# jwcalder/GraphLearningLayer

Hardware: NVIDIA B200
Metric: gll_fwd_bwd_calls_per_sec (higher is better)
Workload: dtype f32

## Files before the change

### graphlearninglayer_b200/csrc/knn.cu

```cuda
#include <math.h>
#include <stdlib.h>
#include <string.h>

#include <algorithm>
#include <vector>

#include <cuda_fp16.h>
#include <cuda_fp16.h>

#include "common.cuh"
#include "knn_common.cuh"

namespace gll {
namespace {

constexpr int BM = 128, BN = 128, BK = 16, PAD = 4;
constexpr int GEMM_THREADS = 256;
constexpr int LDS_A = BM + PAD, LDS_B = BN + PAD;

constexpr size_t gemm_smem_bytes() {
  return sizeof(float) * (2 * BK * LDS_A + 2 * BK * LDS_B) + sizeof(u64) * (BM * KC + BM * BN) +
         sizeof(float) * BM + sizeof(int) * BM;
}

// ... 190 lines not shown
  float* Bs = As + 2 * BK * LDS_A;
  u64* topk = reinterpret_cast<u64*>(Bs + 2 * BK * LDS_B);
  u64* pend = topk + BM * KC;
  float* thr = reinterpret_cast<float*>(pend + BM * BN);
  int* pcnt = reinterpret_cast<int*>(thr + BM);

  const int tid = threadIdx.x, lane = tid & 31, warp = tid >> 5;
  const int tx = tid & 15, ty = tid >> 4;
  const int row0 = row_begin + blockIdx.x * BM;
  const int split = blockIdx.y;
  int t_lo = 0, t_hi = n;
  if (SEG) {
    t_lo = __ldg(&win[row0].x);
    t_hi = __ldg(&win[min(row_end, row0 + BM) - 1].y);
  }
  const int c_begin = t_lo + split * cols_per_split;
  const int c_end = min(t_hi, c_begin + cols_per_split);

  for (int t = tid; t < BM * KC; t += GEMM_THREADS) topk[t] = KEY_INF;
  for (int t = tid; t < BM; t += GEMM_THREADS) {
    thr[t] = INFINITY;
    pcnt[t] = 0;
  }
  __syncthreads();

  const int ktiles = (d + BK - 1) / BK;
  for (int c0 = c_begin; c0 < c_end; c0 += BN) {
    float acc[8][8];
#pragma unroll
    for (int i = 0; i < 8; ++i)
#pragma unroll
      for (int j = 0; j < 8; ++j) acc[i][j] = 0.f;

    float4 ra[2], rb[2];
    load_tile_regs<VEC4>(X, n, d, row0, 0, tid, ra);
    load_tile_regs<VEC4>(X, n, d, c0, 0, tid, rb);
    store_tile_smem(As, LDS_A, tid, ra);
    store_tile_smem(Bs, LDS_B, tid, rb);
    __syncthreads();
    for (int kt = 0; kt < ktiles; ++kt) {
      const int cur = kt & 1;
      if (kt + 1 < ktiles) {
        load_tile_regs<VEC4>(X, n, d, row0, (kt + 1) * BK, tid, ra);
        load_tile_regs<VEC4>(X, n, d, c0, (kt + 1) * BK, tid, rb);
      }
      const float* A = As + cur * BK * LDS_A;
      const float* B = Bs + cur * BK * LDS_B;
#pragma unroll
      for (int kk = 0; kk < BK; ++kk) {
        float4 a0 = *reinterpret_cast<const float4*>(A + kk * LDS_A + ty * 4);
        float4 a1 = *reinterpret_cast<const float4*>(A + kk * LDS_A + 64 + ty * 4);
        float4 b0 = *reinterpret_cast<const float4*>(B + kk * LDS_B + tx * 4);
        float4 b1 = *reinterpret_cast<const float4*>(B + kk * LDS_B + 64 + tx * 4);
        float a[8] = {a0.x, a0.y, a0.z, a0.w, a1.x, a1.y, a1.z, a1.w};
        float b[8] = {b0.x, b0.y, b0.z, b0.w, b1.x, b1.y, b1.z, b1.w};
#pragma unroll
        for (int i = 0; i < 8; ++i)
#pragma unroll
          for (int j = 0; j < 8; ++j) acc[i][j] = fmaf(a[i], b[j], acc[i][j]);
      }
      if (kt + 1 < ktiles) {
        store_tile_smem(As + (cur ^ 1) * BK * LDS_A, LDS_A, tid, ra);
        store_tile_smem(Bs + (cur ^ 1) * BK * LDS_B, LDS_B, tid, rb);
      }
      __syncthreads();
    }

    float sqj[8];
    int gjv[8];
#pragma unroll
    for (int j = 0; j < 8; ++j) {
      int cc = (j < 4) ? tx * 4 + j : 64 + tx * 4 + (j - 4);
      gjv[j] = c0 + cc;
      sqj[j] = (gjv[j] < c_end) ? __ldg(sq + gjv[j]) : 0.f;
    }
#pragma unroll
    for (int i = 0; i < 8; ++i) {
      int rr = (i < 4) ? ty * 4 + i : 64 + ty * 4 + (i - 4);
      int gi = row0 + rr;
      if (gi >= row_end) continue;
      float t = thr[rr];
      float sqi = __ldg(sq + gi);
      int w_lo = 0, w_hi = n;
      if (SEG) {
        const int2 w = __ldg(win + gi);
        w_lo = w.x;
        w_hi = w.y;
      }
#pragma unroll
      for (int j = 0; j < 8; ++j) {
        if (gjv[j] < c_end && gjv[j] != gi && (!SEG || (gjv[j] >= w_lo && gjv[j] < w_hi))) {
          float dist = fmaf(-2.f, acc[i][j], sqi + sqj[j]);
          if (dist < t) {
            int p = atomicAdd(&pcnt[rr], 1);
            pend[rr * BN + p] = make_key(dist, gjv[j]);
          }
        }
      }
    }
    __syncthreads();
    for (int rr = warp * (BM / 8); rr < (warp + 1) * (BM / 8); ++rr) {
      int c = pcnt[rr];
      if (c > 0) {
        u64 mine = topk[rr * KC + lane];
        for (int t = 0; t < c; ++t) list_insert(mine, pend[rr * BN + t], lane);
        topk[rr * KC + lane] = mine;
        if (lane == KC - 1) thr[rr] = (mine == KEY_INF) ? INFINITY : key_dist(mine);
        if (lane == 0) pcnt[rr] = 0;
      }
    }
    __syncthreads();
  }

  for (int rr = warp * (BM / 8); rr < (warp + 1) * (BM / 8); ++rr) {
    int gi = row0 + rr;
    if (gi < row_end) cand[((size_t)gi * splits + split) * KC + lane] = topk[rr * KC + lane];
  }
}

}

namespace {

constexpr int RERANK_WARPS = 4;

template <bool VEC4>
__device__ __forceinline__ double exact_d2(const float* __restrict__ xi_s, const float* __restrict__ xj, int d,
                                           int lane) {
  double part = 0.0;
  if (VEC4) {
    const float4* a = reinterpret_cast<const float4*>(xi_s);
    const float4* b = reinterpret_cast<const float4*>(xj);
    int q = d >> 2;
#pragma unroll 4
    for (int t = lane; t < q; t += 32) {
      float4 u = a[t], v = __ldg(b + t);
      double d0 = (double)u.x - (double)v.x, d1 = (double)u.y - (double)v.y;
      double d2 = (double)u.z - (double)v.z, d3 = (double)u.w - (double)v.w;
      part += d0 * d0;
      part += d1 * d1;
      part += d2 * d2;
      part += d3 * d3;
    }
  } else {
#pragma unroll 4
    for (int t = lane; t < d; t += 32) {
      double df = (double)xi_s[t] - (double)__ldg(xj + t);
      part += df * df;
    }
  }
  return warp_sum(part);
}

__device__ __forceinline__ double exact_d2_reg(const double (&xr)[16], const float* __restrict__ xj, int q, int lane) {
  const float4* b = reinterpret_cast<const float4*>(xj);
  float4 v[4];
#pragma unroll
  for (int t = 0; t < 4; ++t) v[t] = (lane + 32 * t < q) ? __ldg(b + lane + 32 * t) : make_float4(0.f, 0.f, 0.f, 0.f);
  double part = 0.0;
#pragma unroll
  for (int t = 0; t < 4; ++t) {
    if (lane + 32 * t < q) {
      const double d0 = xr[4 * t + 0] - (double)v[t].x, d1 = xr[4 * t + 1] - (double)v[t].y;
      const double d2 = xr[4 * t + 2] - (double)v[t].z, d3 = xr[4 * t + 3] - (double)v[t].w;
      part += d0 * d0;
      part += d1 * d1;
      part += d2 * d2;
      part += d3 * d3;
    }
  }
  return warp_sum(part);
}

__device__ __forceinline__ double knn_err_bound(float err_coef, float sqi, const unsigned* __restrict__ small) {
  const double sqm = (double)__uint_as_float(small[0]), rho = (double)__uint_as_float(small[2]);
  const double xi = sqrt((double)sqi);
  const double rterm = (small[5] == 2u) ? rho * (xi + sqrt(sqm) + rho) : xi * rho;
  return (double)err_coef * ((double)sqi + sqm) + 2.0 * rterm * 1.000001;
}

template <bool VEC4>
__global__ void __launch_bounds__(RERANK_WARPS * 32)
knn_rerank_kernel(const float* __restrict__ X, const float* __restrict__ sq, const unsigned* __restrict__ sqmax_bits,
                  int n, int d, int k, int row_end, CandLayout lay, const u64* __restrict__ cand, float err_coef,
                  int* __restrict__ knn_idx, float* __restrict__ knn_dist, int* __restrict__ flag_count,
                  int* __restrict__ flag_rows, int force_rows) {
  extern __shared__ __align__(16) float xs[];
  const int lane = threadIdx.x & 31, warp = threadIdx.x >> 5;
  const int i = lay.row_begin + blockIdx.x * RERANK_WARPS + warp;
  if (i >= row_end) return;
  float* xi = xs + (size_t)warp * d;
  const bool use_reg = VEC4 && d <= 512;
  double xr[16];
  if (use_reg) {
    const float4* xrow = reinterpret_cast<const float4*>(X + (size_t)i * d);
#pragma unroll
    for (int t = 0; t < 4; ++t) {
      const float4 u = (lane + 32 * t < (d >> 2)) ? __ldg(xrow + lane + 32 * t) : make_float4(0.f, 0.f, 0.f, 0.f);
      xr[4 * t + 0] = (double)u.x;
      xr[4 * t + 1] = (double)u.y;
      xr[4 * t + 2] = (double)u.z;
      xr[4 * t + 3] = (double)u.w;
    }
  } else {
    for (int t = lane; t < d; t += 32) xi[t] = X[(size_t)i * d + t];
  }

  u64 mine = KEY_INF;
  int splits = lay.stride;
  if (lay.tc == 1 || lay.tc == 3) {
    int b0, b1;
    cand_owner_range(lay, (i - lay.row_begin) / lay.row_tile, b0, b1);
    splits = 2 * (b1 - b0 + 1);
  }
  if (splits == 1 && lay.tc == 0) {
    mine = cand[(size_t)i * lay.stride * KC + lane];
  } else {
    for (int s = 0; s < splits; ++s) {
      list_merge_set(mine, cand[((size_t)i * lay.stride + s) * KC + lane], lane);
    }
  }
  u64 last = __shfl_sync(FULL, mine, KC - 1);
  const float lower = (last == KEY_INF) ? INFINITY : key_dist(last);
  __syncwarp();

  const double errb = knn_err_bound(err_coef, sq[i], sqmax_bits);
  const u64 kth = __shfl_sync(FULL, mine, k - 2);
  const float cutoff = (kth == KEY_INF) ? INFINITY : (float)((double)key_dist(kth) + 2.0 * errb + 1e-30) * (1.f + 1e-6f);
  double myd2 = INFINITY;
  int myj = -1;
  for (int c = 0; c < KC; ++c) {
    u64 kc = __shfl_sync(FULL, mine, c);
    if (kc == KEY_INF) break;
    if (c > k - 2 && key_dist(kc) > cutoff) break;
    int j = key_idx(kc);
    double v = use_reg ? exact_d2_reg(xr, X + (size_t)j * d, d >> 2, lane) : exact_d2<VEC4>(xi, X + (size_t)j * d, d, lane);
    if (lane == c) {
      myd2 = v;
      myj = j;
    }
  }
  int rank = 0;
  for (int c = 0; c < KC; ++c) {
    double od = __shfl_sync(FULL, myd2, c);
    int oj = __shfl_sync(FULL, myj, c);
    if (oj >= 0 && (od < myd2 || (od == myd2 && oj < myj))) ++rank;
  }
  if (myj >= 0 && rank < k - 1) {
    knn_idx[(size_t)i * k + 1 + rank] = myj;
    knn_dist[(size_t)i * k + 1 + rank] = (float)sqrt(myd2);
  }
  if (lane == 0) {
    knn_idx[(size_t)i * k] = i;
    knn_dist[(size_t)i * k] = 0.f;
  }
  unsigned who = __ballot_sync(FULL, myj >= 0 && rank == k - 2);
  bool ok = false;
  if (who) {
    double dk = __shfl_sync(FULL, myd2, __ffs(who) - 1);
    ok = ((double)lower - errb > dk) || (lower == INFINITY);
  }
  if (i - lay.row_begin < force_rows) ok = false;
  if (!ok && lane == 0) {
    int p = atomicAdd(flag_count, 1);
    flag_rows[p] = i;
  }
}

constexpr int FB_WARPS = 8;

__device__ __forceinline__ void list_insert_d(double& md, int& mj, double xd, int xj, int lane) {
  bool lt = (md < xd) || (md == xd && mj < xj);
  int pos = __popc(__ballot_sync(FULL, lt));
  double pd = __shfl_up_sync(FULL, md, 1);
  int pj = __shfl_up_sync(FULL, mj, 1);
  if (lane > pos) {
    md = pd;
    mj = pj;
  } else if (lane == pos) {
    md = xd;
    mj = xj;
  }
}

__device__ __forceinline__ bool pair_less(double ad, int aj, double bd, int bj) { return ad < bd || (ad == bd && aj < bj); }
__device__ __forceinline__ void dlist_merge_sorted(double& md, int& mj, double od, int oj, int lane) {
  const double rd = __shfl_sync(FULL, od, 31 - lane);
  const int rj = __shfl_sync(FULL, oj, 31 - lane);
  if (pair_less(rd, rj, md, mj)) {
    md = rd;
    mj = rj;
  }
#pragma unroll
  for (int j = 16; j >= 1; j >>= 1) {
    const double pd = __shfl_xor_sync(FULL, md, j);
    const int pj = __shfl_xor_sync(FULL, mj, j);
    const bool keep_min = (lane & j) == 0;
    const bool p_less = pair_less(pd, pj, md, mj);
    if (p_less == keep_min) {
      md = pd;
      mj = pj;
    }
  }
}

template <bool VEC4>
__global__ void __launch_bounds__(FB_WARPS * 32)
knn_fallback_kernel(const float* __restrict__ X, int n, int d, int k, const int* __restrict__ flag_count,
                    const int* __restrict__ flag_rows, int* __restrict__ knn_idx, float* __restrict__ knn_dist,
                    int* __restrict__ info) {
  extern __shared__ __align__(16) float xs[];
  __shared__ double sd[FB_WARPS][32];
  __shared__ int sj[FB_WARPS][32];
  const int lane = threadIdx.x & 31, warp = threadIdx.x >> 5;
  const int nflag = *flag_count;
  if (blockIdx.x == 0 && threadIdx.x == 0 && info != nullptr) {
    info[GLL_INFO_KNN_FALLBACK_ROWS] = nflag;
    if (nflag > 0) atomicOr(&info[GLL_INFO_STATUS], GLL_STATUS_KNN_FALLBACK);
  }
  for (int f = blockIdx.x; f < nflag; f += gridDim.x) {
    const int i = flag_rows[f];
    for (int t = threadIdx.x; t < d; t += blockDim.x) xs[t] = X[(size_t)i * d + t];
    __syncthreads();
    double ex_d = -1.0;
    int ex_j = -1;
    for (int pass = 0; pass * 32 < k - 1; ++pass) {
      double md = INFINITY;
      int mj = 0x7fffffff;
      for (int j = warp; j < n; j += FB_WARPS) {
        if (j == i) continue;
        double v = exact_d2<VEC4>(xs, X + (size_t)j * d, d, lane);
        if (v > ex_d || (v == ex_d && j > ex_j)) list_insert_d(md, mj, v, j, lane);
      }
      sd[warp][lane] = md;
      sj[warp][lane] = mj;
      __syncthreads();
      if (warp == 0) {
        for (int w = 1; w < FB_WARPS; ++w)
          for (int t = 0; t < 32; ++t) {
            int xj = sj[w][t];
            if (xj == 0x7fffffff) break;
            list_insert_d(md, mj, sd[w][t], xj, lane);
          }
        const int slot = pass * 32 + lane;
        if (slot < k - 1 && mj != 0x7fffffff) {
          knn_idx[(size_t)i * k + 1 + slot] = mj;
          knn_dist[(size_t)i * k + 1 + slot] = (float)sqrt(md);
        }
        if (lane == 0 && pass == 0) {
          knn_idx[(size_t)i * k] = i;
          knn_dist[(size_t)i * k] = 0.f;
        }
        if (lane == 31) {
          sd[0][0] = md;
          sj[0][0] = mj;
        }
      }
      __syncthreads();
      ex_d = sd[0][0];
      ex_j = sj[0][0];
      __syncthreads();
    }
    __syncthreads();
  }
}

template <bool VEC4>
__global__ void __launch_bounds__(FB_WARPS * 32)
knn_fallback_scan_kernel(const float* __restrict__ X, int n, int d, int k, const int* __restrict__ flag_count,
                         const int* __restrict__ flag_rows, int* __restrict__ knn_idx, float* __restrict__ knn_dist,
                         int* __restrict__ info, double* __restrict__ part_d, int* __restrict__ part_j,
                         unsigned* __restrict__ ticket, const int2* __restrict__ win) {
  extern __shared__ __align__(16) float xs[];
  __shared__ double sd[FB_WARPS][32];
  __shared__ int sj[FB_WARPS][32];
  __shared__ int last_cta;
  const int lane = threadIdx.x & 31, warp = threadIdx.x >> 5;
  const int nflag = *flag_count;
  if (blockIdx.x == 0 && threadIdx.x == 0 && info != nullptr) {
    info[GLL_INFO_KNN_FALLBACK_ROWS] = nflag;
    if (nflag > 0) atomicOr(&info[GLL_INFO_STATUS], GLL_STATUS_KNN_FALLBACK);
  }
  if (nflag == 0) return;
  const int G = gridDim.x, C = max(1, min(128, G / nflag));
  const long long T = (long long)nflag * C;
  for (long long t = blockIdx.x; t < T; t += G) {
    const int f = (int)(t / C), c = (int)(t - (long long)f * C);
    const int i = flag_rows[f];
    const int2 w = (win != nullptr) ? win[i] : make_int2(0, n);
    const int j0 = w.x + (int)((long long)(w.y - w.x) * c / C), j1 = w.x + (int)((long long)(w.y - w.x) * (c + 1) / C);
    __syncthreads();
    for (int q = threadIdx.x; q < d; q += blockDim.x) xs[q] = X[(size_t)i * d + q];
    __syncthreads();
    double md = INFINITY, thr_d = INFINITY;
    int mj = 0x7fffffff, thr_j = 0x7fffffff;
    for (int jb = j0 + 4 * warp; jb < j1; jb += 4 * FB_WARPS) {
// ... 59 lines not shown
        }
#pragma unroll
        for (int u = 0; u < 4; ++u) dlist_merge_sorted(md, mj, ld[u], lj[u], lane);
      }
      if (lane < k - 1 && mj != 0x7fffffff) {
        knn_idx[(size_t)i * k + 1 + lane] = mj;
        knn_dist[(size_t)i * k + 1 + lane] = (float)sqrt(md);
      }
      if (lane == 0) {
        knn_idx[(size_t)i * k] = i;
        knn_dist[(size_t)i * k] = 0.f;
      }
    }
    return;
  }
  for (int f = 0; f < nflag; ++f) {
    const int i = flag_rows[f];
    double md = INFINITY;
    int mj = 0x7fffffff;
    for (int c0 = warp; c0 < C; c0 += 4 * FB_WARPS) {
      double ld[4];
      int lj[4];
#pragma unroll
      for (int u = 0; u < 4; ++u) {
        const int c = c0 + u * FB_WARPS;
        ld[u] = (c < C) ? __ldcg(part_d + ((size_t)f * C + c) * 32 + lane) : INFINITY;
        lj[u] = (c < C) ? __ldcg(part_j + ((size_t)f * C + c) * 32 + lane) : 0x7fffffff;
      }
#pragma unroll
      for (int u = 0; u < 4; ++u) dlist_merge_sorted(md, mj, ld[u], lj[u], lane);
    }
    __syncthreads();
    sd[warp][lane] = md;
    sj[warp][lane] = mj;
    __syncthreads();
    if (warp == 0) {
      for (int w = 1; w < FB_WARPS; ++w) dlist_merge_sorted(md, mj, sd[w][lane], sj[w][lane], lane);
      if (lane < k - 1 && mj != 0x7fffffff) {
        knn_idx[(size_t)i * k + 1 + lane] = mj;
        knn_dist[(size_t)i * k + 1 + lane] = (float)sqrt(md);
      }
      if (lane == 0) {
        knn_idx[(size_t)i * k] = i;
        knn_dist[(size_t)i * k] = 0.f;
      }
    }
  }
}


__global__ void __launch_bounds__(RERANK_WARPS * 32)
knn_merge_kernel(int row_end, CandLayout lay, const u64* __restrict__ cand, u64* __restrict__ merged, u64* __restrict__ excl) {
  const int lane = threadIdx.x & 31, warp = threadIdx.x >> 5;
  const int i = lay.row_begin + blockIdx.x * RERANK_WARPS + warp;
  if (i >= row_end) return;
  int splits = lay.stride;
  if (lay.tc == 1) {
    int b0, b1;
    cand_owner_range(lay, (i - lay.row_begin) / lay.row_tile, b0, b1);
    splits = 2 * (b1 - b0 + 1);
  }
  u64 mine = KEY_INF;
  for (int s = 0; s < splits; ++s) {
    list_merge_set(mine, cand[((size_t)i * lay.stride + s) * KC + lane], lane);
  }
  merged[(size_t)(i - lay.row_begin) * KC + lane] = mine;
  if (excl != nullptr && lane == KC - 1) excl[i] = mine;
}

template <bool VEC4>
__global__ void __launch_bounds__(RERANK_WARPS * 32)
knn_rerank64_kernel(const float* __restrict__ X, const float* __restrict__ sq, const unsigned* __restrict__ sqmax_bits, int n, int d,
                    int k, int row_begin, int row_end, const u64* __restrict__ m1, const u64* __restrict__ m2, float err_coef,
                    int* __restrict__ knn_idx, float* __restrict__ knn_dist, int* __restrict__ flag_count,
                    int* __restrict__ flag_rows) {
  extern __shared__ __align__(16) float xs[];
  const int lane = threadIdx.x & 31, warp = threadIdx.x >> 5;
  const int i = row_begin + blockIdx.x * RERANK_WARPS + warp;
  if (i >= row_end) return;
  float* xi = xs + (size_t)warp * d;
  for (int t = lane; t < d; t += 32) xi[t] = X[(size_t)i * d + t];
  __syncwarp();
  const u64 ca = m1[(size_t)(i - row_begin) * KC + lane];
  u64 cb = m2[(size_t)(i - row_begin) * KC + lane];
  const u64 last = __shfl_sync(FULL, cb, KC - 1);
  const float lower = (last == KEY_INF) ? INFINITY : key_dist(last);
  {
    bool dup = false;
    for (int c = 0; c < KC; ++c) {
      const u64 oa = __shfl_sync(FULL, ca, c);
      dup |= (oa != KEY_INF && cb != KEY_INF && key_idx(oa) == key_idx(cb));
    }
    if (dup) cb = KEY_INF;
  }
  double da = INFINITY, db = INFINITY;
  int ja = -1, jb = -1;
  for (int c = 0; c < 2 * KC; ++c) {
    const u64 kc = __shfl_sync(FULL, (c < KC) ? ca : cb, c & (KC - 1));
    if (kc == KEY_INF) continue;
    const int j = key_idx(kc);
    const double v = exact_d2<VEC4>(xi, X + (size_t)j * d, d, lane);
    if (lane == (c & (KC - 1))) {
      if (c < KC) {
        da = v;
        ja = j;
      } else {
        db = v;
        jb = j;
      }
    }
  }
  int ra = 0, rb = 0;
  for (int c = 0; c < 2 * KC; ++c) {
    const double od = __shfl_sync(FULL, (c < KC) ? da : db, c & (KC - 1));
    const int oj = __shfl_sync(FULL, (c < KC) ? ja : jb, c & (KC - 1));
    if (oj < 0) continue;
    ra += (od < da || (od == da && oj < ja)) ? 1 : 0;
    rb += (od < db || (od == db && oj < jb)) ? 1 : 0;
  }
  if (ja >= 0 && ra < k - 1) {
    knn_idx[(size_t)i * k + 1 + ra] = ja;
    knn_dist[(size_t)i * k + 1 + ra] = (float)sqrt(da);
  }
  if (jb >= 0 && rb < k - 1) {
    knn_idx[(size_t)i * k + 1 + rb] = jb;
    knn_dist[(size_t)i * k + 1 + rb] = (float)sqrt(db);
  }
  if (lane == 0) {
    knn_idx[(size_t)i * k] = i;
    knn_dist[(size_t)i * k] = 0.f;
  }
  const unsigned wa = __ballot_sync(FULL, ja >= 0 && ra == k - 2), wb = __ballot_sync(FULL, jb >= 0 && rb == k - 2);
  bool ok = false;
  if (wa | wb) {
    const double dk = wa ? __shfl_sync(FULL, da, __ffs(wa) - 1) : __shfl_sync(FULL, db, __ffs(wb) - 1);
    const double errb = knn_err_bound(err_coef, sq[i], sqmax_bits);
    ok = ((double)lower - errb > dk) || (lower == INFINITY);
  }
  if (!ok && lane == 0) {
    int p = atomicAdd(flag_count, 1);
    flag_rows[p] = i;
  }
}

}

int knn_fallback_grid() { return 2 * device_info().sms; }
size_t knn_fallback_scratch_bytes() { return align_up((size_t)knn_fallback_grid() * 32 * (sizeof(double) + sizeof(int)), 256); }

int knn_finish(const float* X, const float* sq, const unsigned* sqmax_bits, int n, int d, int k, int row_begin, int row_end,
               CandLayout lay, const u64* cand, float err_coef, int* knn_idx, float* knn_dist, int* flag_count, int* flag_rows,
               int* info, void* fb_scratch, cudaStream_t st, const int2* win) {
  const bool vec4 = (d % 4 == 0) && ((reinterpret_cast<uintptr_t>(X) & 15) == 0);
  size_t smem = sizeof(float) * (size_t)RERANK_WARPS * d;
  lay.row_begin = row_begin;
  int blocks = ceil_div(row_end - row_begin, RERANK_WARPS);
  int force_rows = 0;
  if (const char* e = getenv("GLL_B200_KNN_FORCE_FALLBACK")) force_rows = atoi(e);
  if (vec4) {
    if (smem > 48 * 1024)
      GLL_CUDA_CHECK(cudaFuncSetAttribute(knn_rerank_kernel<true>, cudaFuncAttributeMaxDynamicSharedMemorySize, (int)smem));
    {
      GLL_PROF(KID_RERANK, st);
      knn_rerank_kernel<true><<<blocks, RERANK_WARPS * 32, smem, st>>>(X, sq, sqmax_bits, n, d, k, row_end, lay, cand,
                                                                      err_coef, knn_idx, knn_dist, flag_count, flag_rows, force_rows);
    }
  } else {
    if (smem > 48 * 1024)
      GLL_CUDA_CHECK(cudaFuncSetAttribute(knn_rerank_kernel<false>, cudaFuncAttributeMaxDynamicSharedMemorySize, (int)smem));
    {
      GLL_PROF(KID_RERANK, st);
      knn_rerank_kernel<false><<<blocks, RERANK_WARPS * 32, smem, st>>>(X, sq, sqmax_bits, n, d, k, row_end, lay, cand,
                                                                       err_coef, knn_idx, knn_dist, flag_count, flag_rows, force_rows);
    }
  }
  GLL_LAUNCH_CHECK();
  size_t fsmem = sizeof(float) * (size_t)d;
  if (getenv("GLL_B200_KNN_DEBUG") != nullptr) return GLL_OK;
  {
    const int fblocks = knn_fallback_grid();
    double* part_d = reinterpret_cast<double*>(fb_scratch);
    int* part_j = reinterpret_cast<int*>(part_d + (size_t)fblocks * 32);
    unsigned* ticket = reinterpret_cast<unsigned*>(flag_count) + 7;
    GLL_PROF(KID_KNN_FALLBACK, st);
    if (vec4)
      knn_fallback_scan_kernel<true><<<fblocks, FB_WARPS * 32, fsmem, st>>>(X, n, d, k, flag_count, flag_rows, knn_idx, knn_dist, info,
                                                                           part_d, part_j, ticket, win);
    else
      knn_fallback_scan_kernel<false><<<fblocks, FB_WARPS * 32, fsmem, st>>>(X, n, d, k, flag_count, flag_rows, knn_idx, knn_dist, info,
                                                                            part_d, part_j, ticket, win);
  }
  GLL_LAUNCH_CHECK();
  return GLL_OK;
}

static int knn_finish64(const float* X, const float* sq, const unsigned* sqmax_bits, int n, int d, int k, int row_begin, int row_end,
                       const u64* m1, const u64* m2, float err_coef, int* knn_idx, float* knn_dist, int* flag_count,
                       int* flag_rows, int* info, cudaStream_t st) {
  const bool vec4 = (d % 4 == 0) && ((reinterpret_cast<uintptr_t>(X) & 15) == 0);
  const size_t smem = sizeof(float) * (size_t)RERANK_WARPS * d;
  const int blocks = ceil_div(row_end - row_begin, RERANK_WARPS);
  {
    GLL_PROF(KID_RERANK, st);
    if (vec4) {
      if (smem > 48 * 1024)
        GLL_CUDA_CHECK(cudaFuncSetAttribute(knn_rerank64_kernel<true>, cudaFuncAttributeMaxDynamicSharedMemorySize, (int)smem));
      knn_rerank64_kernel<true><<<blocks, RERANK_WARPS * 32, smem, st>>>(X, sq, sqmax_bits, n, d, k, row_begin, row_end, m1, m2,
                                                                          err_coef, knn_idx, knn_dist, flag_count, flag_rows);
    } else {
      if (smem > 48 * 1024)
        GLL_CUDA_CHECK(cudaFuncSetAttribute(knn_rerank64_kernel<false>, cudaFuncAttributeMaxDynamicSharedMemorySize, (int)smem));
      knn_rerank64_kernel<false><<<blocks, RERANK_WARPS * 32, smem, st>>>(X, sq, sqmax_bits, n, d, k, row_begin, row_end, m1, m2,
                                                                           err_coef, knn_idx, knn_dist, flag_count, flag_rows);
    }
  }
  GLL_LAUNCH_CHECK();
  const size_t fsmem = sizeof(float) * (size_t)d;
  const int fblocks = device_info().sms;
  if (getenv("GLL_B200_KNN_DEBUG") != nullptr) return GLL_OK;
  {
    GLL_PROF(KID_KNN_FALLBACK, st);
    if (vec4)
      knn_fallback_kernel<true><<<fblocks, FB_WARPS * 32, fsmem, st>>>(X, n, d, k, flag_count, flag_rows, knn_idx, knn_dist, info);
    else
      knn_fallback_kernel<false><<<fblocks, FB_WARPS * 32, fsmem, st>>>(X, n, d, k, flag_count, flag_rows, knn_idx, knn_dist, info);
  }
  GLL_LAUNCH_CHECK();
  return GLL_OK;
}

static int simt_splits(int n, int rows, int* cols_per_split) {
  int row_tiles = ceil_div(rows, BM), col_tiles = ceil_div(n, BN);
  int want = ceil_div(2 * device_info().sms, row_tiles);
  want = max(1, min(want, min(col_tiles, KNN_MAX_SPLITS)));
  int tiles_per = ceil_div(col_tiles, want);
  *cols_per_split = tiles_per * BN;
  return ceil_div(col_tiles, tiles_per);
}

static int cand_stride(int n, int d, int row_begin, int row_end) {
  const TcPlan plan = knn_tc_plan(n, d, row_begin, row_end);
  if (plan.ok) return plan.max_splits;
  int cps;
  return simt_splits(n, row_end - row_begin, &cps);
}

static size_t knn_common_bytes(int n, int d, size_t rows, int stride) {
  size_t b = 0;
  b += align_up(sizeof(float) * (size_t)n, 256);
  b += 256;
  b += align_up(sizeof(u64) * rows * (size_t)stride * KC, 256);
  b += align_up(sizeof(int) * rows, 256);
  b += knn_tc_ws_upper(n, d);
  b += align_up(sizeof(unsigned) * (size_t)n, 256);
  b += align_up(sizeof(float) * (size_t)n, 256);
  b += knn_fallback_scratch_bytes() + 256;
  return b;
}

size_t knn_ws_bytes(int n, int d, int k, int row_begin, int row_end) {
  const size_t rows = (size_t)(row_end - row_begin);
  size_t b = knn_common_bytes(n, d, rows, cand_stride(n, d, row_begin, row_end));
  if (k > KC + 1) b += 2 * align_up(sizeof(u64) * rows * KC, 256) + align_up(sizeof(u64) * (size_t)n, 256);
  return b + 1024;
}

namespace {

struct KnnBufs {
  float* sq;
  unsigned* small;
  int* flag_count;
  u64* cand;
  int* flag_rows;
  char* tc_ws;
  unsigned* thr_g;
  float* rscale;
  void* fb_scratch;
};

KnnBufs knn_carve(Carver& cv, int n, int d, int row_begin, int row_end, int stride) {
  const int rows = row_end - row_begin;
  KnnBufs b;
  b.sq = cv.take<float>(n);
  b.small = cv.take<unsigned>(64);
  b.flag_count = reinterpret_cast<int*>(b.small + 1);
  b.cand = cv.take<u64>((size_t)rows * stride * KC) - (size_t)row_begin * stride * KC;
  b.flag_rows = cv.take<int>(rows);
  b.tc_ws = cv.take<char>(knn_tc_ws_upper(n, d));
  b.thr_g = cv.take<unsigned>(n);
  b.rscale = cv.take<float>(n);
  b.fb_scratch = cv.take<char>(knn_fallback_scratch_bytes());
  const char* sh = getenv("GLL_B200_KNN_SHARE");
  if (sh && sh[0] == '0') b.thr_g = nullptr;
  return b;
}

CandLayout layout_of(const TcPlan& plan, int row_begin, const int* gfirst = nullptr) {
  CandLayout lay;
  lay.stride = plan.max_splits;
  lay.tc = plan.aligned ? 2 : (gfirst != nullptr ? 3 : 1);
  lay.row_tile = 128 * plan.rstep;
  lay.col_tiles = plan.col_tiles;
  lay.grid = plan.grid;
  lay.units = plan.units;
  lay.row_begin = row_begin;
  lay.gfirst = gfirst;
  return lay;
}

CandLayout simt_layout(int splits) {
  CandLayout lay;
  lay.stride = splits;
  lay.tc = 0;
  lay.row_tile = lay.col_tiles = lay.grid = 0;
  lay.units = 0;
  lay.row_begin = 0;
  lay.gfirst = nullptr;
  return lay;
}

float simt_err_coef(int d) {
  const double u = 5.9604644775390625e-8;
  return (float)(((double)d * u / (1.0 - (double)d * u) + 4.0 * u) * 1.0001);
}

int launch_simt(const float* X, const float* sq, int n, int d, int cps, int splits, u64* cand, int row_begin, int row_end,
                const int2* win, cudaStream_t st) {
  const bool vec4 = (d % 4 == 0) && ((reinterpret_cast<uintptr_t>(X) & 15) == 0);
  const bool seg = win != nullptr;
  auto kern = vec4 ? (seg ? knn_gemm_topk_kernel<true, true> : knn_gemm_topk_kernel<true, false>)
                   : (seg ? knn_gemm_topk_kernel<false, true> : knn_gemm_topk_kernel<false, false>);
  const dim3 grid(ceil_div(row_end - row_begin, BM), splits);
  const size_t smem = gemm_smem_bytes();
  GLL_CUDA_CHECK(set_max_dynamic_smem_once((const void*)kern, (int)smem));
  {
    GLL_PROF(KID_GRAM_TOPK, st);
    kern<<<grid, GEMM_THREADS, smem, st>>>(X, sq, n, d, cps, splits, cand, row_begin, row_end, win);
  }
  GLL_LAUNCH_CHECK();
  return GLL_OK;
}

}

static int launch_split_f16(const float* X, int n, int d, const TcPlan& plan, float* sq, unsigned* small, char* tc_ws, float* rscale,
                            unsigned* thr_g, cudaStream_t st) {
  __half* H = reinterpret_cast<__half*>(tc_ws);
  __half* L = (plan.passes == 2) ? reinterpret_cast<__half*>(tc_ws + align_up((size_t)n * plan.d_pad * 2, 256)) : nullptr;
  const int grid = ceil_div((long long)ceil_div(n, plan.d_pad <= 1024 ? 2 : 1) * 32, 256);
  if (plan.d_pad <= 256)
    sqnorm_split_f16_kernel<4><<<grid, 256, 0, st>>>(X, n, d, plan.d_pad, sq, small, H, L, rscale, thr_g);
  else if (plan.d_pad <= 512)
    sqnorm_split_f16_kernel<8><<<grid, 256, 0, st>>>(X, n, d, plan.d_pad, sq, small, H, L, rscale, thr_g);
  else if (plan.d_pad <= 1024)
    sqnorm_split_f16_kernel<16><<<grid, 256, 0, st>>>(X, n, d, plan.d_pad, sq, small, H, L, rscale, thr_g);
  else
    sqnorm_split_f16_kernel<0><<<grid, 256, 0, st>>>(X, n, d, plan.d_pad, sq, small, H, L, rscale, thr_g);
  GLL_LAUNCH_CHECK();
  return GLL_OK;
}

static int launch_norms(const float* X, int n, int d, const TcPlan& plan, const KnnBufs& b, cudaStream_t st) {
  GLL_PROF(KID_SQNORM, st);
  if (plan.ok) return launch_split_f16(X, n, d, plan, b.sq, b.small, b.tc_ws, b.rscale, b.thr_g, st);
  sqnorm_kernel<<<ceil_div((long long)n * 32, 256), 256, 0, st>>>(X, n, d, b.sq, b.small);
  GLL_LAUNCH_CHECK();
  return GLL_OK;
}

int knn_debug_gram_tile(const float* X, int n, int d, int row_tile, int col_tile, float* acc_out, float* rscale_out, void* ws,
                        size_t ws_bytes, cudaStream_t st) {
  GLL_REQUIRE(X && acc_out && rscale_out && ws, "null pointer");
  GLL_REQUIRE(n >= 256 && d >= 1, "the tensor-core path needs n >= 256");
  if (ws_bytes < knn_ws_bytes(n, d, 25, 0, n)) {
    set_error("workspace too small: %zu < %zu", ws_bytes, knn_ws_bytes(n, d, 25, 0, n));
    return GLL_ERR_WORKSPACE;
  }
  const TcPlan plan = knn_tc_plan(n, d, 0, n);
  GLL_REQUIRE(plan.ok, "tensor-core plan not available for this shape");
  GLL_REQUIRE(row_tile >= 0 && row_tile * 128 < n && col_tile >= 0 && col_tile * 256 < n, "tile out of range");
  Carver cv(ws, ws_bytes);
  float* sq = cv.take<float>(n);
  unsigned* small = cv.take<unsigned>(64);
  char* tc_ws = cv.take<char>(knn_tc_ws_upper(n, d));
  float* rscale = cv.take<float>(n);
  GLL_CUDA_CHECK(cudaMemsetAsync(small, 0, 256, st));
  const int rcs = launch_split_f16(X, n, d, plan, sq, small, tc_ws, rscale, nullptr, st);
  if (rcs) return rcs;
  GLL_CUDA_CHECK(cudaMemcpyAsync(rscale_out, rscale, sizeof(float) * (size_t)n, cudaMemcpyDeviceToDevice, st));
  return knn_tc_debug_tile(plan, n, tc_ws, row_tile, col_tile, acc_out, st);
}

int knn_run(const float* X, int n, int d, int k, int row_begin, int row_end, int* knn_idx, float* knn_dist, int* info,
            void* ws, size_t ws_bytes, cudaStream_t st) {
  GLL_REQUIRE(X && knn_idx && knn_dist && ws, "null pointer");
  GLL_REQUIRE(n >= k && k >= 2 && k <= 2 * KC, "need n >= k and 2 <= k <= 64");
  GLL_REQUIRE(d >= 1, "d must be positive");
  GLL_REQUIRE(0 <= row_begin && row_begin < row_end && row_end <= n, "bad row range");
  if (ws_bytes < knn_ws_bytes(n, d, k, row_begin, row_end)) {
    set_error("kNN workspace too small: %zu < %zu", ws_bytes, knn_ws_bytes(n, d, k, row_begin, row_end));
    return GLL_ERR_WORKSPACE;
  }
  const int rows = row_end - row_begin;
  Carver cv(ws, ws_bytes);
  const KnnBufs kb = knn_carve(cv, n, d, row_begin, row_end, cand_stride(n, d, row_begin, row_end));
  float* sq = kb.sq;
  unsigned* small = kb.small;
  unsigned* sqmax_bits = small;
  int* flag_count = kb.flag_count;
  u64* cand = kb.cand;
  int* flag_rows = kb.flag_rows;
  char* tc_ws = kb.tc_ws;
  unsigned* thr_g = kb.thr_g;
  float* rscale = kb.rscale;

  CandLayout lay;
  float err_coef;
  const TcPlan plan = knn_tc_plan(n, d, row_begin, row_end);
  GLL_CUDA_CHECK(cudaMemsetAsync(small, 0, 256, st));
  {
    const int rcs = launch_norms(X, n, d, plan, kb, st);
    if (rcs) return rcs;
  }

  if (k > KC + 1) {
    GLL_REQUIRE(plan.ok, "k > 33 needs the tensor-core path (n >= 256, row range starting on a multiple of 128)");
    u64* merged1 = cv.take<u64>((size_t)rows * KC);
    u64* merged2 = cv.take<u64>((size_t)rows * KC);
    u64* excl = cv.take<u64>(n);
    lay = layout_of(plan, row_begin);
    const int mblocks = ceil_div(rows, RERANK_WARPS);
    int rc = knn_tc_candidates(X, sq, rscale, small, n, d, row_end, plan, tc_ws, cand, nullptr, thr_g, st);
    if (rc) return rc;
    {
      GLL_PROF(KID_RERANK, st);
      knn_merge_kernel<<<mblocks, RERANK_WARPS * 32, 0, st>>>(row_end, lay, cand, merged1, excl);
    }
    GLL_LAUNCH_CHECK();
    rc = knn_tc_candidates(X, sq, rscale, small, n, d, row_end, plan, tc_ws, cand, excl, nullptr, st);
    if (rc) return rc;
    {
      GLL_PROF(KID_RERANK, st);
      knn_merge_kernel<<<mblocks, RERANK_WARPS * 32, 0, st>>>(row_end, lay, cand, merged2, nullptr);
    }
    GLL_LAUNCH_CHECK();
    return knn_finish64(X, sq, sqmax_bits, n, d, k, row_begin, row_end, merged1, merged2, knn_tc_err_coef(d, plan.passes), knn_idx, knn_dist,
                        flag_count, flag_rows, info, st);
  }
  if (plan.ok) {
    int rc = knn_tc_candidates(X, sq, rscale, small, n, d, row_end, plan, tc_ws, cand, nullptr, thr_g, st);
    if (rc) return rc;
    lay = layout_of(plan, row_begin);
    err_coef = knn_tc_err_coef(d, plan.passes);
  } else {
    int cps;
    const int splits = simt_splits(n, rows, &cps);
    const int rc = launch_simt(X, sq, n, d, cps, splits, cand, row_begin, row_end, nullptr, st);
    if (rc) return rc;
    lay = simt_layout(splits);
    err_coef = simt_err_coef(d);
  }
  return knn_finish(X, sq, sqmax_bits, n, d, k, row_begin, row_end, lay, cand, err_coef, knn_idx, knn_dist, flag_count, flag_rows,
                    info, kb.fb_scratch, st);
}


namespace {

// ... 288 lines not shown
```

### graphlearninglayer_b200/csrc/knn_common.cuh

```cuda
#pragma once
#include <vector>

#include "common.cuh"

namespace gll {

typedef unsigned long long u64;
constexpr int KC = 32;
constexpr int KNN_MAX_SPLITS = 32;
constexpr u64 KEY_INF = ~0ull;

__device__ __forceinline__ u64 make_key(float dist, int j) {
  return ((u64)float_to_ordered(dist) << 32) | (uint32_t)j;
}
__device__ __forceinline__ float key_dist(u64 k) { return ordered_to_float((uint32_t)(k >> 32)); }
__device__ __forceinline__ int key_idx(u64 k) { return (int)(uint32_t)k; }

__device__ __forceinline__ void list_insert(u64& mine, u64 x, int lane) {
  int pos = __popc(__ballot_sync(FULL, mine < x));
  u64 prev = __shfl_up_sync(FULL, mine, 1);
  if (lane > pos)
    mine = prev;
  else if (lane == pos)
    mine = x;
}

__device__ __forceinline__ void key_cmpx(u64& k, int j, bool keep_min) {
  const u64 o = __shfl_xor_sync(FULL, k, j);
  const bool less = k < o;
  k = (less == keep_min) ? k : o;
}
__device__ __forceinline__ void key_sort32(u64& k, int lane) {
#pragma unroll
  for (int w = 2; w <= 32; w <<= 1) {
#pragma unroll
    for (int j = w >> 1; j >= 1; j >>= 1) {
      const bool up = (lane & w) == 0;
      key_cmpx(k, j, ((lane & j) == 0) == up);
    }
  }
}
__device__ __forceinline__ void list_merge_set(u64& mine, u64 c, int lane) {
  unsigned m = __ballot_sync(FULL, c < __shfl_sync(FULL, mine, KC - 1));
  if (m == 0) return;
  if (__popc(m) > 6) {
    key_sort32(c, lane);
    const u64 r = __shfl_sync(FULL, c, 31 - lane);
    mine = (r < mine) ? r : mine;
#pragma unroll
    for (int j = 16; j >= 1; j >>= 1) key_cmpx(mine, j, (lane & j) == 0);
    return;
  }
  while (m) {
    const int t = __ffs(m) - 1;
    m &= m - 1;
    const u64 x = __shfl_sync(FULL, c, t);
    if (x < __shfl_sync(FULL, mine, KC - 1)) list_insert(mine, x, lane);
  }
}

struct TcPlan {
  int ok, d_pad, kblocks, row_tiles, col_tiles, grid, max_splits, rt0, aligned, rstep;
  int ct0, col_begin;
  int passes;
  long long units;
  size_t ws_bytes;
};

struct SegDev {
  const int2* win;
  const int* gfirst;
  const int* gct;
  const int* bstart;
};

TcPlan knn_tc_plan(int n, int d, int row_begin, int row_end, int col_begin = 0);
TcPlan knn_tc_plan_segments(int n, int d, const int* seg_ptr, int nseg, std::vector<int>* tab);
size_t knn_tc_ws_upper(int n, int d);
int knn_tc_candidates(const float* X, const float* sq, const float* rscale, const unsigned* small, int n, int d, int row_end, const TcPlan& plan,
                      void* tc_ws, u64* cand, const u64* excl, unsigned* thr_g, cudaStream_t st, const SegDev* seg = nullptr);
float knn_tc_err_coef(int d, int passes);
int knn_tc_debug_tile(const TcPlan& plan, int n, void* tc_ws, int rt, int ct, float* acc_out, cudaStream_t st);

struct CandLayout {
  int stride;
  int tc;
  int row_begin;
  int row_tile, col_tiles, grid;
  long long units;
  const int* gfirst;
};

__device__ __forceinline__ void cand_owner_range(const CandLayout& lay, long long rt, int& b0, int& b1) {
  const long long f0 = (lay.tc == 3) ? (long long)__ldg(lay.gfirst + rt) : rt * lay.col_tiles;
  const long long f1 = (lay.tc == 3) ? (long long)__ldg(lay.gfirst + rt + 1) : (rt + 1) * lay.col_tiles;
  b0 = (int)(((f0 + 1) * lay.grid - 1) / lay.units);
  b1 = (int)((f1 * lay.grid - 1) / lay.units);
}

int knn_finish(const float* X, const float* sq, const unsigned* sqmax_bits, int n, int d, int k, int row_begin, int row_end,
               CandLayout lay,
               const u64* cand, float err_coef, int* knn_idx, float* knn_dist, int* flag_count, int* flag_rows,
               int* info, void* fb_scratch, cudaStream_t st, const int2* win = nullptr);

}
```

Before: 2259.

## Pipeline kNN rerank candidate loads with cp.async ring and grouped warp reductions

Reworks the rerank kernel so candidate rows are prefetched into a per-warp shared-memory ring with cp.async while earlier candidates are processed. Partial distances for four candidates are reduced together with a butterfly that shares shuffles. The candidate count is computed once by ballot instead of an early-break loop, split candidate loads are software-prefetched, and the 64-bit division in cand_owner_range becomes a reciprocal multiply. The ring triples dynamic shared memory per warp, which may lower occupancy, and adds wait-group synchronisation.

```diff
diff --git a/graphlearninglayer_b200/csrc/knn.cu b/graphlearninglayer_b200/csrc/knn.cu
--- a/graphlearninglayer_b200/csrc/knn.cu
+++ b/graphlearninglayer_b200/csrc/knn.cu
@@ -366,24 +366,62 @@
   return warp_sum(part);
 }
 
-__device__ __forceinline__ double exact_d2_reg(const double (&xr)[16], const float* __restrict__ xj, int q, int lane) {
-  const float4* b = reinterpret_cast<const float4*>(xj);
-  float4 v[4];
-#pragma unroll
-  for (int t = 0; t < 4; ++t) v[t] = (lane + 32 * t < q) ? __ldg(b + lane + 32 * t) : make_float4(0.f, 0.f, 0.f, 0.f);
+constexpr int RERANK_RING = 3;
+
+__device__ __forceinline__ void ring_fetch(float4* slot, const float4* __restrict__ xj, int q, int lane) {
+#pragma unroll
+  for (int t = 0; t < 4; ++t) {
+    const int c = lane + 32 * t;
+    if (c < q) {
+      const unsigned dst = (unsigned)__cvta_generic_to_shared(slot + c);
+      asm volatile("cp.async.cg.shared.global [%0], [%1], 16;\n" ::"r"(dst), "l"(xj + c) : "memory");
+    }
+  }
+}
+__device__ __forceinline__ void ring_commit() { asm volatile("cp.async.commit_group;\n" ::: "memory"); }
+template <int N>
+__device__ __forceinline__ void ring_wait() { asm volatile("cp.async.wait_group %0;\n" ::"n"(N) : "memory"); }
+__device__ __forceinline__ void ring_wait_all() { asm volatile("cp.async.wait_all;\n" ::: "memory"); }
+
+__device__ __forceinline__ double ring_part(const double (&xr)[16], const float4* slot, int q, int lane) {
   double part = 0.0;
 #pragma unroll
   for (int t = 0; t < 4; ++t) {
     if (lane + 32 * t < q) {
-      const double d0 = xr[4 * t + 0] - (double)v[t].x, d1 = xr[4 * t + 1] - (double)v[t].y;
-      const double d2 = xr[4 * t + 2] - (double)v[t].z, d3 = xr[4 * t + 3] - (double)v[t].w;
+      const float4 v = slot[lane + 32 * t];
+      const double d0 = xr[4 * t + 0] - (double)v.x, d1 = xr[4 * t + 1] - (double)v.y;
+      const double d2 = xr[4 * t + 2] - (double)v.z, d3 = xr[4 * t + 3] - (double)v.w;
       part += d0 * d0;
       part += d1 * d1;
       part += d2 * d2;
       part += d3 * d3;
     }
   }
-  return warp_sum(part);
+  return part;
+}
+
+constexpr int RERANK_GROUP = 4;
+__device__ __forceinline__ double warp_sum_group(double (&p)[RERANK_GROUP], int lane) {
+#pragma unroll
+  for (int o = 16, m = RERANK_GROUP; m > 1; o >>= 1, m >>= 1) {
+    const bool up = (lane & o) != 0;
+#pragma unroll
+    for (int t = 0; t < m / 2; ++t) {
+      const double keep = up ? p[t + m / 2] : p[t], send = up ? p[t] : p[t + m / 2];
+      p[t] = keep + __shfl_xor_sync(FULL, send, o);
+    }
+  }
+  double v = p[0];
+#pragma unroll
+  for (int o = 16 / RERANK_GROUP; o > 0; o >>= 1) v += __shfl_xor_sync(FULL, v, o);
+  return v;
+}
+__device__ __forceinline__ int rerank_group_lane(int g) {
+  int src = 0;
+#pragma unroll
+  for (int o = 16, m = RERANK_GROUP; m > 1; o >>= 1, m >>= 1)
+    if (g & (m / 2)) src |= o;
+  return src;
 }
 
 __device__ __forceinline__ double knn_err_bound(float err_coef, float sqi, const unsigned* __restrict__ small) {
@@ -403,10 +441,10 @@
   const int lane = threadIdx.x & 31, warp = threadIdx.x >> 5;
   const int i = lay.row_begin + blockIdx.x * RERANK_WARPS + warp;
   if (i >= row_end) return;
+  const bool use_ring = VEC4 && d <= 512;
   float* xi = xs + (size_t)warp * d;
-  const bool use_reg = VEC4 && d <= 512;
   double xr[16];
-  if (use_reg) {
+  if (use_ring) {
     const float4* xrow = reinterpret_cast<const float4*>(X + (size_t)i * d);
 #pragma unroll
     for (int t = 0; t < 4; ++t) {
@@ -430,8 +468,12 @@
   if (splits == 1 && lay.tc == 0) {
     mine = cand[(size_t)i * lay.stride * KC + lane];
   } else {
+    const u64* crow = cand + (size_t)i * lay.stride * KC + lane;
+    u64 next = crow[0];
     for (int s = 0; s < splits; ++s) {
-      list_merge_set(mine, cand[((size_t)i * lay.stride + s) * KC + lane], lane);
+      const u64 cur = next;
+      if (s + 1 < splits) next = crow[(size_t)(s + 1) * KC];
+      list_merge_set(mine, cur, lane);
     }
   }
   u64 last = __shfl_sync(FULL, mine, KC - 1);
@@ -441,21 +483,59 @@
   const double errb = knn_err_bound(err_coef, sq[i], sqmax_bits);
   const u64 kth = __shfl_sync(FULL, mine, k - 2);
   const float cutoff = (kth == KEY_INF) ? INFINITY : (float)((double)key_dist(kth) + 2.0 * errb + 1e-30) * (1.f + 1e-6f);
+  const unsigned take = __ballot_sync(FULL, mine != KEY_INF && (unsigned)key_idx(mine) < (unsigned)n &&
+                                                (lane <= k - 2 || !(key_dist(mine) > cutoff)));
+  const int ncand = (take == FULL) ? KC : __ffs(~take) - 1;
   double myd2 = INFINITY;
   int myj = -1;
-  for (int c = 0; c < KC; ++c) {
-    u64 kc = __shfl_sync(FULL, mine, c);
-    if (kc == KEY_INF) break;
-    if (c > k - 2 && key_dist(kc) > cutoff) break;
-    int j = key_idx(kc);
-    double v = use_reg ? exact_d2_reg(xr, X + (size_t)j * d, d >> 2, lane) : exact_d2<VEC4>(xi, X + (size_t)j * d, d, lane);
-    if (lane == c) {
-      myd2 = v;
-      myj = j;
+  if (use_ring) {
+    const int q = d >> 2;
+    float4* ring = reinterpret_cast<float4*>(xs) + (size_t)warp * RERANK_RING * q;
+    const float4* X4 = reinterpret_cast<const float4*>(X);
+#pragma unroll
+    for (int c = 0; c < RERANK_RING - 1; ++c) {
+      const int j = key_idx(__shfl_sync(FULL, mine, c));
+      if (c < ncand) ring_fetch(ring + c * q, X4 + (size_t)j * q, q, lane);
+      ring_commit();
+    }
+    int slot = 0;
+    for (int c0 = 0; c0 < ncand; c0 += RERANK_GROUP) {
+      double p[RERANK_GROUP];
+#pragma unroll
+      for (int u = 0; u < RERANK_GROUP; ++u) {
+        const int c = c0 + u;
+        p[u] = 0.0;
+        if (c < ncand) {
+          const int cf = c + RERANK_RING - 1;
+          const int jf = key_idx(__shfl_sync(FULL, mine, cf & (KC - 1)));
+          if (cf < ncand) ring_fetch(ring + (slot == 0 ? RERANK_RING - 1 : slot - 1) * q, X4 + (size_t)jf * q, q, lane);
+          ring_commit();
+          ring_wait<RERANK_RING - 1>();
+          p[u] = ring_part(xr, ring + slot * q, q, lane);
+          slot = (slot == RERANK_RING - 1) ? 0 : slot + 1;
+        }
+      }
+      const double sum = warp_sum_group(p, lane);
+      const int g = lane - c0;
+      const double v = __shfl_sync(FULL, sum, rerank_group_lane(g & (RERANK_GROUP - 1)));
+      if (g >= 0 && g < RERANK_GROUP && lane < ncand) {
+        myd2 = v;
+        myj = key_idx(mine);
+      }
+    }
+    ring_wait_all();
+  } else {
+    for (int c = 0; c < ncand; ++c) {
+      const int j = key_idx(__shfl_sync(FULL, mine, c));
+      const double v = exact_d2<VEC4>(xi, X + (size_t)j * d, d, lane);
+      if (lane == c) {
+        myd2 = v;
+        myj = j;
+      }
     }
   }
   int rank = 0;
-  for (int c = 0; c < KC; ++c) {
+  for (int c = 0; c < ncand; ++c) {
     double od = __shfl_sync(FULL, myd2, c);
     int oj = __shfl_sync(FULL, myj, c);
     if (oj >= 0 && (od < myd2 || (od == myd2 && oj < myj))) ++rank;
@@ -821,22 +901,20 @@
                CandLayout lay, const u64* cand, float err_coef, int* knn_idx, float* knn_dist, int* flag_count, int* flag_rows,
                int* info, void* fb_scratch, cudaStream_t st, const int2* win) {
   const bool vec4 = (d % 4 == 0) && ((reinterpret_cast<uintptr_t>(X) & 15) == 0);
-  size_t smem = sizeof(float) * (size_t)RERANK_WARPS * d;
+  const size_t smem = sizeof(float) * (size_t)RERANK_WARPS * d * ((vec4 && d <= 512) ? RERANK_RING : 1);
   lay.row_begin = row_begin;
   int blocks = ceil_div(row_end - row_begin, RERANK_WARPS);
   int force_rows = 0;
   if (const char* e = getenv("GLL_B200_KNN_FORCE_FALLBACK")) force_rows = atoi(e);
   if (vec4) {
-    if (smem > 48 * 1024)
-      GLL_CUDA_CHECK(cudaFuncSetAttribute(knn_rerank_kernel<true>, cudaFuncAttributeMaxDynamicSharedMemorySize, (int)smem));
+    GLL_CUDA_CHECK(set_max_dynamic_smem_once((const void*)knn_rerank_kernel<true>, (int)smem));
     {
       GLL_PROF(KID_RERANK, st);
       knn_rerank_kernel<true><<<blocks, RERANK_WARPS * 32, smem, st>>>(X, sq, sqmax_bits, n, d, k, row_end, lay, cand,
                                                                       err_coef, knn_idx, knn_dist, flag_count, flag_rows, force_rows);
     }
   } else {
-    if (smem > 48 * 1024)
-      GLL_CUDA_CHECK(cudaFuncSetAttribute(knn_rerank_kernel<false>, cudaFuncAttributeMaxDynamicSharedMemorySize, (int)smem));
+    GLL_CUDA_CHECK(set_max_dynamic_smem_once((const void*)knn_rerank_kernel<false>, (int)smem));
     {
       GLL_PROF(KID_RERANK, st);
       knn_rerank_kernel<false><<<blocks, RERANK_WARPS * 32, smem, st>>>(X, sq, sqmax_bits, n, d, k, row_end, lay, cand,
@@ -973,6 +1051,7 @@
   lay.col_tiles = plan.col_tiles;
   lay.grid = plan.grid;
   lay.units = plan.units;
+  lay.units_rcp = plan.units > 0 ? ~0ull / (u64)plan.units : 0;
   lay.row_begin = row_begin;
   lay.gfirst = gfirst;
   return lay;
@@ -984,6 +1063,7 @@
   lay.tc = 0;
   lay.row_tile = lay.col_tiles = lay.grid = 0;
   lay.units = 0;
+  lay.units_rcp = 0;
   lay.row_begin = 0;
   lay.gfirst = nullptr;
   return lay;
diff --git a/graphlearninglayer_b200/csrc/knn_common.cuh b/graphlearninglayer_b200/csrc/knn_common.cuh
--- a/graphlearninglayer_b200/csrc/knn_common.cuh
+++ b/graphlearninglayer_b200/csrc/knn_common.cuh
@@ -88,14 +88,21 @@
   int row_begin;
   int row_tile, col_tiles, grid;
   long long units;
+  u64 units_rcp;
   const int* gfirst;
 };
+
+__device__ __forceinline__ long long div_units(const CandLayout& lay, long long a) {
+  u64 q = __umul64hi((u64)a, lay.units_rcp);
+  if ((u64)a - q * (u64)lay.units >= (u64)lay.units) ++q;
+  return (long long)q;
+}
 
 __device__ __forceinline__ void cand_owner_range(const CandLayout& lay, long long rt, int& b0, int& b1) {
   const long long f0 = (lay.tc == 3) ? (long long)__ldg(lay.gfirst + rt) : rt * lay.col_tiles;
   const long long f1 = (lay.tc == 3) ? (long long)__ldg(lay.gfirst + rt + 1) : (rt + 1) * lay.col_tiles;
-  b0 = (int)(((f0 + 1) * lay.grid - 1) / lay.units);
-  b1 = (int)((f1 * lay.grid - 1) / lay.units);
+  b0 = (int)div_units(lay, (f0 + 1) * lay.grid - 1);
+  b1 = (int)div_units(lay, f1 * lay.grid - 1);
 }
 
 int knn_finish(const float* X, const float* sq, const unsigned* sqmax_bits, int n, int d, int k, int row_begin, int row_end,
```

After: 2347, median of 6. 3.9% higher.
